# cfdeinza/reinforcement-learning-rendezvous

Hardware: AMD Instinct MI355X
Metric: env steps/sec (higher is better)
Workload: dtype f64

## Files before the change

### reinforcement_learning_rendezvous_amd/csrc/rdv_policy.h

```cpp
#pragma once

#include <hip/hip_runtime.h>
#include <stdint.h>

#include <cmath>
#include <cstring>
#include <vector>

#include "rdv_device.h"

namespace rdv {

constexpr int kPolIn = 17, kPolHid = 64, kPolOut = 6;
constexpr int kPolWaveEnvs = 32;
constexpr int kPolBlock = 512;
constexpr int kPolBlockEnvs = (kPolBlock / 64) * kPolWaveEnvs;

typedef float f32x16 __attribute__((ext_vector_type(16)));
typedef float pol_f4 __attribute__((ext_vector_type(4)));
typedef float pol_f2 __attribute__((ext_vector_type(2)));
typedef _Float16 f16x8 __attribute__((ext_vector_type(8)));

constexpr int kPolXShift = 10;
constexpr int kPolFragBytes = 64 * 16;
constexpr int kPolW1Frag = 0, kPolW2Frag = 8, kPolW3Frag = 24, kPolFrags = 32;
constexpr int kPolF32 = kPolFrags * kPolFragBytes / 4;
constexpr int kPolB1 = kPolF32, kPolB2 = kPolB1 + 64, kPolB3 = kPolB2 + 64, kPolStd = kPolB3 + 32, kPolLogStd = kPolStd + 8,
              kPolScale = kPolLogStd + 8, kPolFloats = kPolScale + 4;
static_assert(kPolFloats % 4 == 0, "the parameter block is copied as float4");
constexpr int kPolObsStage = kPolWaveEnvs * kPolIn, kPolActStage = kPolWaveEnvs * kPolOut;
constexpr int kPolLdsBytes = (kPolFloats + (kPolBlock / 64) * (kPolObsStage + kPolActStage)) * 4;

inline uint16_t pol_f16_rn(float x) {
  uint32_t u; std::memcpy(&u, &x, 4);
  const uint32_t sign = (u >> 16) & 0x8000u;
  const uint32_t a = u & 0x7fffffffu;
  if (a > 0x7f800000u) return (uint16_t)(sign | 0x7e00u);
  if (a >= 0x477ff000u) return (uint16_t)(sign | 0x7c00u);
  if (a < 0x33000001u) return (uint16_t)sign;
  int e = (int)(a >> 23) - 127;
  uint32_t m = (a & 0x7fffffu) | 0x800000u;
  int shift = e >= -14 ? 13 : 13 + (-14 - e);
  uint32_t q = m >> shift;
  const uint32_t rem = m & ((1u << shift) - 1u), half = 1u << (shift - 1);
  if (rem > half || (rem == half && (q & 1u))) ++q;
  uint32_t out = e >= -14 ? (uint32_t)((e + 15) << 10) + (q - 0x400u) : q;
  return (uint16_t)(sign | out);
}
inline float pol_f16_f(uint16_t hbits) {
  const uint32_t sign = (uint32_t)(hbits & 0x8000u) << 16, e = (hbits >> 10) & 0x1fu, m = hbits & 0x3ffu;
  float mag;
  if (e == 0) mag = std::ldexp((float)m, -24);
  else if (e == 31) mag = m ? NAN : INFINITY;
  else mag = std::ldexp((float)(m | 0x400u), (int)e - 25);
  return sign ? -mag : mag;
}
inline int pol_layer_shift(const float* wts, int count) {
  float mx = 0.0f;
  for (int i = 0; i < count; ++i) mx = std::fmax(mx, std::fabs(wts[i]));
  int sft = 10;
  while (sft > -20 && std::ldexp(mx, sft) >= 32768.0f) --sft;
  return sft;
}
inline void pol_put(uint16_t* frags, int frag0, int mt_count, int ks_count, int mt, int ks, int lane, int j, float wv, int sft) {
  const float ws = std::ldexp(wv, sft);
  const uint16_t hi = pol_f16_rn(ws);
  const uint16_t term[2] = {hi, pol_f16_rn(ws - pol_f16_f(hi))};
  for (int q = 0; q < 2; ++q) frags[((size_t)(frag0 + (q * mt_count + mt) * ks_count + ks) * 64 + (size_t)lane) * 8 + (size_t)j] = term[q];
}

inline void pack_policy_weights(const float* w1, const float* b1, const float* w2, const float* b2, const float* w3, const float* b3,
                                const float* log_std, int out_dim, std::vector<float>& packed) {
  packed.assign((size_t)kPolFloats, 0.0f);
  uint16_t* frags = reinterpret_cast<uint16_t*>(packed.data());
  const int sh1 = pol_layer_shift(w1, kPolHid * kPolIn), sh2 = pol_layer_shift(w2, kPolHid * kPolHid), sh3 = pol_layer_shift(w3, out_dim * kPolHid);
  auto put = [&](int frag0, int mt_count, int ks_count, int mt, int ks, int lane, int j, float wv, int sft) {
    pol_put(frags, frag0, mt_count, ks_count, mt, ks, lane, j, wv, sft);
  };
  for (int lane = 0; lane < 64; ++lane) {
    const int r = lane & 31, h = lane >> 5;
    for (int j = 0; j < 8; ++j) {
      for (int mt = 0; mt < 2; ++mt) {
        for (int s = 0; s < 2; ++s) {
          const int k = 16 * s + 8 * h + j;
          put(kPolW1Frag, 2, 2, mt, s, lane, j, k < kPolIn ? w1[(32 * mt + r) * kPolIn + k] : 0.0f, sh1);
        }
        for (int ks = 0; ks < 4; ++ks) {
          const int k = 32 * (ks >> 1) + 16 * (ks & 1) + 8 * (j >> 2) + 4 * h + (j & 3);
          put(kPolW2Frag, 2, 4, mt, ks, lane, j, w2[(32 * mt + r) * kPolHid + k], sh2);
        }
      }
      for (int ks = 0; ks < 4; ++ks) {
        const int k = 32 * (ks >> 1) + 16 * (ks & 1) + 8 * (j >> 2) + 4 * h + (j & 3);
        put(kPolW3Frag, 1, 4, 0, ks, lane, j, r < out_dim ? w3[r * kPolHid + k] : 0.0f, sh3);
      }
    }
  }
  const float acc1 = std::ldexp(1.0f, kPolXShift + sh1), acc2 = std::ldexp(1.0f, kPolXShift + sh2), acc3 = std::ldexp(1.0f, kPolXShift + sh3);
  for (int mt = 0; mt < 2; ++mt)
    for (int h = 0; h < 2; ++h)
      for (int e = 0; e < 16; ++e) {
        const int row = (e & 3) + 8 * (e >> 2) + 4 * h;
        packed[kPolB1 + (mt * 2 + h) * 16 + e] = b1[32 * mt + row] * acc1;
        packed[kPolB2 + (mt * 2 + h) * 16 + e] = b2[32 * mt + row] * acc2;
        if (mt == 0) packed[kPolB3 + h * 16 + e] = row < out_dim ? b3[row] * acc3 : 0.0f;
      }
  packed[kPolScale + 0] = 1.0f / acc1; packed[kPolScale + 1] = 1.0f / acc2; packed[kPolScale + 2] = 1.0f / acc3;
  if (log_std) for (int j = 0; j < out_dim; ++j) { packed[kPolStd + j] = std::exp(log_std[j]); packed[kPolLogStd + j] = log_std[j]; }
}

__device__ __forceinline__ void tanh2_f32(float x0, float x1, float kexp, float& t0, float& t1) {
  const pol_f2 x = {x0, x1};
  const pol_f2 y = x * kexp;
  const pol_f2 e = {__builtin_amdgcn_exp2f(y.x), __builtin_amdgcn_exp2f(y.y)};
  const pol_f2 s1 = e + 1.0f;
  const pol_f2 r = {__builtin_amdgcn_rcpf(s1.x), __builtin_amdgcn_rcpf(s1.y)};
  constexpr float one = (float)(1 << kPolXShift);
  const pol_f2 t = __builtin_elementwise_fma(pol_f2{-2.0f * one, -2.0f * one}, r, pol_f2{one, one});
  t0 = t.x; t1 = t.y;
}

__device__ __forceinline__ void box_muller(uint32_t a, uint32_t b, float& n0, float& n1) {
  const float u1 = ((float)(a >> 8) + 0.5f) * (1.0f / 16777216.0f);
  const float u2 = ((float)(b >> 8) + 0.5f) * (1.0f / 16777216.0f);
  const float r = sqrtf(-2.0f * __logf(u1));
  float s, c;
  __sincosf(6.28318530717958647692f * u2, &s, &c);
  n0 = r * c; n1 = r * s;
}

__device__ __forceinline__ void wave_fence() {
  __builtin_amdgcn_fence(__ATOMIC_ACQ_REL, "wavefront");
  __builtin_amdgcn_wave_barrier();
}

typedef _Float16 pol_h2 __attribute__((ext_vector_type(2)));
__device__ __forceinline__ void split2(const float (&x)[8], f16x8 (&t)[2]) {
  uint32_t hi[4], lo[4];
#pragma unroll
  for (int p = 0; p < 4; ++p) {
    const pol_f2 v = {x[2 * p], x[2 * p + 1]};
    const pol_h2 h = __builtin_convertvector(v, pol_h2);
    __builtin_memcpy(&hi[p], &h, 4);
  }
  asm("v_fma_mixlo_f16 %0, %4, 1.0, -%12 op_sel_hi:[0,0,1]\n\t"
      "v_fma_mixlo_f16 %1, %6, 1.0, -%13 op_sel_hi:[0,0,1]\n\t"
      "v_fma_mixlo_f16 %2, %8, 1.0, -%14 op_sel_hi:[0,0,1]\n\t"
      "v_fma_mixlo_f16 %3, %10, 1.0, -%15 op_sel_hi:[0,0,1]\n\t"
      "v_fma_mixhi_f16 %0, %5, 1.0, -%12 op_sel:[0,0,1] op_sel_hi:[0,0,1]\n\t"
      "v_fma_mixhi_f16 %1, %7, 1.0, -%13 op_sel:[0,0,1] op_sel_hi:[0,0,1]\n\t"
      "v_fma_mixhi_f16 %2, %9, 1.0, -%14 op_sel:[0,0,1] op_sel_hi:[0,0,1]\n\t"
      "v_fma_mixhi_f16 %3, %11, 1.0, -%15 op_sel:[0,0,1] op_sel_hi:[0,0,1]\n\t"
      "s_nop 0"
      : "=&v"(lo[0]), "=&v"(lo[1]), "=&v"(lo[2]), "=&v"(lo[3])
      : "v"(x[0]), "v"(x[1]), "v"(x[2]), "v"(x[3]), "v"(x[4]), "v"(x[5]), "v"(x[6]), "v"(x[7]), "v"(hi[0]), "v"(hi[1]), "v"(hi[2]), "v"(hi[3]));
#pragma unroll
  for (int p = 0; p < 4; ++p) {
    pol_h2 h, l;
    __builtin_memcpy(&h, &hi[p], 4);
    __builtin_memcpy(&l, &lo[p], 4);
    t[0][2 * p] = h.x; t[0][2 * p + 1] = h.y; t[1][2 * p] = l.x; t[1][2 * p + 1] = l.y;
  }
}

__device__ __forceinline__ f32x16 mfma3(const f16x8 (&a)[2], const f16x8 (&b)[2], f32x16 d) {
  d = __builtin_amdgcn_mfma_f32_32x32x16_f16(a[1], b[0], d, 0, 0, 0);
  d = __builtin_amdgcn_mfma_f32_32x32x16_f16(a[0], b[1], d, 0, 0, 0);
  d = __builtin_amdgcn_mfma_f32_32x32x16_f16(a[0], b[0], d, 0, 0, 0);
  return d;
}

template <int MT, int KS>
__device__ __forceinline__ void layer(const float* w, int frag0, const float* biasp, const f16x8 (&xb)[KS][2], int lane, f32x16 (&d)[MT]) {
  const f16x8* wf = reinterpret_cast<const f16x8*>(w) + lane;
  const int h = lane >> 5;
#pragma unroll
  for (int mt = 0; mt < MT; ++mt)
#pragma unroll
    for (int e4 = 0; e4 < 4; ++e4) {
      const float4 b = *reinterpret_cast<const float4*>(biasp + (mt * 2 + h) * 16 + 4 * e4);
      d[mt][4 * e4 + 0] = b.x; d[mt][4 * e4 + 1] = b.y; d[mt][4 * e4 + 2] = b.z; d[mt][4 * e4 + 3] = b.w;
    }
#pragma unroll
  for (int mt = 0; mt < MT; ++mt)
#pragma unroll
    for (int ks = 0; ks < KS; ++ks) {
      f16x8 a[2];
#pragma unroll
      for (int q = 0; q < 2; ++q) a[q] = wf[(frag0 + (q * MT + mt) * KS + ks) * 64];
      d[mt] = mfma3(a, xb[ks], d[mt]);
    }
}

__device__ __forceinline__ void activate(const f32x16& d, float kexp, f16x8 (&lo_step)[2], f16x8 (&hi_step)[2]) {
  float x[8];
#pragma unroll
  for (int j = 0; j < 8; j += 2) tanh2_f32(d[j], d[j + 1], kexp, x[j], x[j + 1]);
  split2(x, lo_step);
#pragma unroll
  for (int j = 0; j < 8; j += 2) tanh2_f32(d[8 + j], d[9 + j], kexp, x[j], x[j + 1]);
  split2(x, hi_step);
}

__device__ __forceinline__ void actor_inputs(const float* rows, int lane, f16x8 (&x0)[2][2]) {
  const int r = lane & 31, h = lane >> 5;
  const float* row = rows + r * kPolIn;
  constexpr float xs = (float)(1 << kPolXShift), xmax = 63.0f * xs;
  auto in = [&](float v) { const float c = __builtin_amdgcn_fmed3f(v * xs, -xmax, xmax); return v != v ? v : c; };
  {
    float x[8];
#pragma unroll
    for (int j = 0; j < 8; ++j) x[j] = in(row[8 * h + j]);
    split2(x, x0[0]);
    const float last = in(row[16]);
#pragma unroll
    for (int j = 0; j < 8; ++j) x[j] = 0.0f;
    x[0] = h == 0 ? last : 0.0f;
    split2(x, x0[1]);
  }
}

__device__ __forceinline__ void actor_means(const float* w, const float* rows, int lane, float (&mean)[4]) {
  f16x8 x0[2][2];
  actor_inputs(rows, lane, x0);
  constexpr float two_log2e = 2.8853900817779268f;
  f32x16 d1[2];
  layer<2, 2>(w, kPolW1Frag, w + kPolB1, x0, lane, d1);
  f16x8 x1[4][2];
  const float k1 = two_log2e * w[kPolScale + 0];
  activate(d1[0], k1, x1[0], x1[1]);
  activate(d1[1], k1, x1[2], x1[3]);
  f32x16 d2[2];
  layer<2, 4>(w, kPolW2Frag, w + kPolB2, x1, lane, d2);
  f16x8 x2[4][2];
  const float k2 = two_log2e * w[kPolScale + 1];
  activate(d2[0], k2, x2[0], x2[1]);
  activate(d2[1], k2, x2[2], x2[3]);
  f32x16 d3[1];
  layer<1, 4>(w, kPolW3Frag, w + kPolB3, x2, lane, d3);
  const float s3 = w[kPolScale + 2];
  mean[0] = d3[0][0] * s3; mean[1] = d3[0][1] * s3; mean[2] = d3[0][2] * s3; mean[3] = d3[0][3] * s3;
}

__device__ __forceinline__ void actor_noise(int lane, uint64_t seed, uint64_t id, uint64_t counter, float (&z)[4]) {
  const int h = lane >> 5;
  uint32_t c0 = (uint32_t)id, c1 = (uint32_t)(id >> 32), c2 = (uint32_t)counter, c3 = (uint32_t)(counter >> 32) * 2u + (uint32_t)h;
  philox4x32_10(c0, c1, c2, c3, (uint32_t)seed, (uint32_t)(seed >> 32) ^ 0x504F4C49u);
  box_muller(c0, c1, z[0], z[1]);
  box_muller(c2, c3, z[2], z[3]);
}

__device__ __forceinline__ float actor_apply_at(const float* sd, int lane, const float (&z)[4], float (&a)[4]) {
  const int h = lane >> 5;
  float lp = 0.0f;
#pragma unroll
  for (int c = 0; c < 4; ++c) {
    const bool valid = h == 0 || c < 2;
    a[c] = fmaf(sd[4 * h + c], z[c], a[c]);
    lp += valid ? fmaf(-0.5f * z[c], z[c], -sd[kPolLogStd - kPolStd + 4 * h + c]) : 0.0f;
  }
  return (lp + __shfl_xor(lp, 32)) - 5.5136312f;
}
__device__ __forceinline__ float actor_apply(const float* w, int lane, const float (&z)[4], float (&a)[4]) {
  return actor_apply_at(w + kPolStd, lane, z, a);
}
__device__ __forceinline__ float actor_sample_at(const float* sd, int lane, int deterministic, uint64_t seed, uint64_t id, uint64_t counter,
                                                 float (&a)[4]) {
  float z[4] = {0.0f, 0.0f, 0.0f, 0.0f};
  if (!deterministic) actor_noise(lane, seed, id, counter, z);
  return actor_apply_at(sd, lane, z, a);
}

__device__ __forceinline__ float clip_action(float v) { return (v != v) ? v : fminf(fmaxf(v, -1.0f), 1.0f); }

__device__ __forceinline__ void stage_obs_rows(const float* __restrict__ obs, int64_t wave_base, int64_t nrows, float* rows, int lane) {
  if (nrows > 0) {
    const float* src = obs + wave_base * kPolIn;
    if (nrows == kPolWaveEnvs) {
#pragma unroll
      for (int k = 0; k < 3; ++k) {
        const int q = k * 64 + lane;
        if (q < kPolObsStage / 4)
          *reinterpret_cast<pol_f4*>(rows + 4 * q) = __builtin_nontemporal_load(reinterpret_cast<const pol_f4*>(src + 4 * q));
      }
    } else {
      const int64_t valid = nrows * kPolIn;
      for (int j = 0; j < 9; ++j) {
        const int idx = j * 64 + lane;
        if (idx < kPolObsStage) rows[idx] = idx < valid ? src[idx] : 0.0f;
      }
    }
  }
}

__device__ __forceinline__ void actor_outputs(const float* sd, int lane, int64_t wave_base, int64_t nrows, int deterministic, uint64_t seed,
                                              uint64_t counter, uint64_t env_id_offset, float (&a)[4], float* arows, float* __restrict__ actions,
                                              float* __restrict__ raw_actions, float* __restrict__ log_prob) {
  const int r = lane & 31, h = lane >> 5;
  const float logp = actor_sample_at(sd, lane, deterministic, seed, env_id_offset + (uint64_t)(wave_base + r), counter, a);
  if (log_prob && h == 0 && r < nrows) log_prob[wave_base + r] = logp;
  if (raw_actions && r < nrows) {
    float* dst = raw_actions + (wave_base + r) * kPolOut + 4 * h;
    dst[0] = a[0]; dst[1] = a[1];
    if (h == 0) { dst[2] = a[2]; dst[3] = a[3]; }
  }

  if (h == 0) {
#pragma unroll
    for (int c = 0; c < 4; ++c) arows[r * kPolOut + c] = clip_action(a[c]);
  } else {
    arows[r * kPolOut + 4] = clip_action(a[0]);
    arows[r * kPolOut + 5] = clip_action(a[1]);
  }
  wave_fence();
  {
    float* dst = actions + wave_base * kPolOut;
    const int64_t valid = nrows * kPolOut;
#pragma unroll
    for (int k = 0; k < 2; ++k) {
      const int idx = k * 128 + lane * 2;
      if (idx + 1 < valid) {
        *reinterpret_cast<float2*>(dst + idx) = *reinterpret_cast<const float2*>(arows + idx);
      } else if (idx < valid) {
        dst[idx] = arows[idx];
      }
    }
  }
}

#ifndef RDV_POLICY_FUNCTIONS_ONLY
__global__ __launch_bounds__(kPolBlock) void policy_act_kernel(const float* __restrict__ W, const float* __restrict__ obs,
                                                               float* __restrict__ actions, int64_t n, int deterministic,
                                                               uint64_t seed, uint64_t counter, uint64_t env_id_offset,
                                                               float* __restrict__ raw_actions, float* __restrict__ log_prob) {
  extern __shared__ __attribute__((aligned(16))) float lds[];
  float* w = lds;
  const int lane = threadIdx.x & 63;
  const int wv = threadIdx.x >> 6;
  float* rows = lds + kPolFloats + wv * kPolObsStage;
  float* arows = lds + kPolFloats + (kPolBlock / 64) * kPolObsStage + wv * kPolActStage;
  const int64_t wave_base = ((int64_t)blockIdx.x * (kPolBlock / 64) + wv) * kPolWaveEnvs;
  const int64_t nrows = (n - wave_base) < kPolWaveEnvs ? (n - wave_base) : kPolWaveEnvs;

#ifndef RDV_POL_NOSTAGE
  for (int q = threadIdx.x; q < kPolFloats / 4; q += kPolBlock)
    *reinterpret_cast<float4*>(w + 4 * q) = *reinterpret_cast<const float4*>(W + 4 * q);
#endif

  stage_obs_rows(obs, wave_base, nrows, rows, lane);
  __syncthreads();
  if (nrows <= 0) return;

  float a[4];
  if (wv < 4) __builtin_amdgcn_s_setprio(1);
  actor_means(w, rows, lane, a);
  if (wv < 4) __builtin_amdgcn_s_setprio(0);
  actor_outputs(w + kPolStd, lane, wave_base, nrows, deterministic, seed, counter, env_id_offset, a, arows, actions, raw_actions, log_prob);
}

__global__ __launch_bounds__(kPolBlock) void policy_value_kernel(const float* __restrict__ W, const float* __restrict__ obs,
                                                                 float* __restrict__ values, int64_t n) {
  extern __shared__ __attribute__((aligned(16))) float lds[];
  float* w = lds;
  const int lane = threadIdx.x & 63;
  const int wv = threadIdx.x >> 6;
  float* rows = lds + kPolFloats + wv * kPolObsStage;
  const int64_t wave_base = ((int64_t)blockIdx.x * (kPolBlock / 64) + wv) * kPolWaveEnvs;
  const int64_t nrows = (n - wave_base) < kPolWaveEnvs ? (n - wave_base) : kPolWaveEnvs;
  for (int q = threadIdx.x; q < kPolFloats / 4; q += kPolBlock)
    *reinterpret_cast<float4*>(w + 4 * q) = *reinterpret_cast<const float4*>(W + 4 * q);
  stage_obs_rows(obs, wave_base, nrows, rows, lane);
  __syncthreads();
  if (nrows <= 0) return;
  float v[4];
  actor_means(w, rows, lane, v);
  if (lane < nrows) values[wave_base + lane] = v[0];
}
#endif

}
```

### reinforcement_learning_rendezvous_amd/csrc/rdv_policy_mlp.h

```cpp
#pragma once

#include "rdv_policy.h"
#include "../../include/rdv.h"

namespace rdv {

constexpr float kMlpSigmoidAbsErr = 2.0e-7f;
constexpr int kMlpLayers = RDV_MLP_MAX_HIDDEN + 1;
constexpr int kMlpRec = 8, kMlpRecStride = 8, kMlpStd = 48, kMlpZero = 64, kMlpHdr = 128;
static_assert(kPolLogStd - kPolStd == 8, "actor_apply_at reads log_std 8 floats behind exp(log_std)");
constexpr int kMlpStageFloats = (kPolBlock / 64) * (kPolObsStage + kPolActStage);
constexpr int kMlpMaxFloats = kMlpHdr + (8 + 3 * 16 + 8) * (kPolFragBytes / 4) + (4 * 2 + 1) * 32;
constexpr int kMlpMaxLdsBytes = (kMlpMaxFloats + kMlpStageFloats) * 4;
static_assert(kMlpMaxLdsBytes <= 160 * 1024, "the largest network's workgroup must fit the CU's 160 KiB of LDS");
inline int mlp_lds_bytes(int block_floats) { return (block_floats + kMlpStageFloats) * 4; }

inline int mlp_tiles(int width) { return width == 64 ? 2 : 1; }
inline int mlp_ksteps(int width) { return width / 16; }

inline void pack_mlp_weights(const RdvMlpSpec& spec, int out_dim, const float* const* weights, const float* const* biases,
                             const float* log_std, std::vector<float>& packed) {
  const int L = spec.n_hidden;
  int frag0[kMlpLayers], mt_n[kMlpLayers], ks_n[kMlpLayers], in_w[kMlpLayers], out_w[kMlpLayers], frags_total = 0, tiles_total = 0;
  for (int l = 0; l <= L; ++l) {
    in_w[l] = l == 0 ? kPolIn : spec.hidden[l - 1];
    out_w[l] = l < L ? spec.hidden[l] : out_dim;
    mt_n[l] = l < L ? mlp_tiles(out_w[l]) : 1;
    ks_n[l] = l == 0 ? 2 : mlp_ksteps(in_w[l]);
    frag0[l] = frags_total;
    frags_total += 2 * mt_n[l] * ks_n[l];
    tiles_total += mt_n[l];
  }
  const int bias0 = kMlpHdr + frags_total * (kPolFragBytes / 4);
  const int total = bias0 + tiles_total * 32;
  packed.assign((size_t)total, 0.0f);
  int32_t* hdr = reinterpret_cast<int32_t*>(packed.data());
  hdr[0] = L; hdr[1] = spec.activation; hdr[2] = out_dim; hdr[3] = total;
  uint16_t* frags = reinterpret_cast<uint16_t*>(packed.data() + kMlpHdr);
  int bias_at = bias0;
  for (int l = 0; l <= L; ++l) {
    const float* wl = weights[l];
    const int sft = pol_layer_shift(wl, out_w[l] * in_w[l]);
    for (int lane = 0; lane < 64; ++lane) {
      const int r = lane & 31, h = lane >> 5;
      for (int j = 0; j < 8; ++j)
        for (int mt = 0; mt < mt_n[l]; ++mt)
          for (int ks = 0; ks < ks_n[l]; ++ks) {
            const int k = l == 0 ? 16 * ks + 8 * h + j : 32 * (ks >> 1) + 16 * (ks & 1) + 8 * (j >> 2) + 4 * h + (j & 3);
            const int row = 32 * mt + r;
            pol_put(frags, frag0[l], mt_n[l], ks_n[l], mt, ks, lane, j, (row < out_w[l] && k < in_w[l]) ? wl[row * in_w[l] + k] : 0.0f, sft);
          }
    }
    const float acc = std::ldexp(1.0f, kPolXShift + sft);
    for (int mt = 0; mt < mt_n[l]; ++mt)
      for (int h = 0; h < 2; ++h)
        for (int e = 0; e < 16; ++e) {
          const int row = 32 * mt + (e & 3) + 8 * (e >> 2) + 4 * h;
          packed[(size_t)(bias_at + (mt * 2 + h) * 16 + e)] = row < out_w[l] ? biases[l][row] * acc : 0.0f;
        }
    int32_t* rec = hdr + kMlpRec + kMlpRecStride * l;
    rec[0] = frag0[l]; rec[1] = bias_at; rec[2] = mt_n[l]; rec[3] = ks_n[l];
    packed[(size_t)(kMlpRec + kMlpRecStride * l + 4)] = 1.0f / acc;
    bias_at += mt_n[l] * 32;
  }
  if (log_std) for (int j = 0; j < out_dim; ++j) { packed[kMlpStd + j] = std::exp(log_std[j]); packed[kMlpStd + 8 + j] = log_std[j]; }
}

hipError_t mlp_raise_lds_limit();
void mlp_launch_act(int activation, const float* W, int block_floats, const float* obs, float* actions, int64_t n, int deterministic,
                    uint64_t seed, uint64_t counter, uint64_t env_id_offset, float* raw_actions, float* log_prob, hipStream_t s);
void mlp_launch_value(int activation, const float* W, int block_floats, const float* obs, float* values, int64_t n, hipStream_t s);

template <int ACT>
__device__ __forceinline__ float mlp_act_const(float inv) {
  if (ACT == RDV_ACT_TANH) return 2.8853900817779268f * inv;
  if (ACT == RDV_ACT_SIGMOID) return -1.4426950408889634f * inv;
  return inv * (float)(1 << kPolXShift);
}

template <int ACT>
__device__ __forceinline__ void mlp_act2(float x0, float x1, float k, float& t0, float& t1) {
  constexpr float one = (float)(1 << kPolXShift);
  if (ACT == RDV_ACT_TANH) {
    tanh2_f32(x0, x1, k, t0, t1);
  } else if (ACT == RDV_ACT_SIGMOID) {
    const pol_f2 y = pol_f2{x0, x1} * k;
    const pol_f2 e = {__builtin_amdgcn_exp2f(y.x), __builtin_amdgcn_exp2f(y.y)};
    const pol_f2 s1 = e + 1.0f;
    const pol_f2 r = {__builtin_amdgcn_rcpf(s1.x), __builtin_amdgcn_rcpf(s1.y)};
    const pol_f2 t = r * one;
    t0 = t.x; t1 = t.y;
  } else {
    const pol_f2 v = pol_f2{x0, x1} * k;
    const float c0 = __builtin_amdgcn_fmed3f(v.x, 0.0f, 63.0f * one), c1 = __builtin_amdgcn_fmed3f(v.y, 0.0f, 63.0f * one);
    t0 = v.x != v.x ? v.x : c0; t1 = v.y != v.y ? v.y : c1;
  }
}

template <int ACT>
__device__ __forceinline__ void mlp_activate(const f32x16& d, float k, f16x8 (&lo_step)[2], f16x8 (&hi_step)[2]) {
  float x[8];
#pragma unroll
  for (int j = 0; j < 8; j += 2) mlp_act2<ACT>(d[j], d[j + 1], k, x[j], x[j + 1]);
  split2(x, lo_step);
#pragma unroll
  for (int j = 0; j < 8; j += 2) mlp_act2<ACT>(d[8 + j], d[9 + j], k, x[j], x[j + 1]);
  split2(x, hi_step);
}

__device__ __forceinline__ void mlp_add_bias(f32x16& d, const float* b16) {
#pragma unroll
  for (int e4 = 0; e4 < 4; ++e4) {
    const float4 b = *reinterpret_cast<const float4*>(b16 + 4 * e4);
    d[4 * e4 + 0] += b.x; d[4 * e4 + 1] += b.y; d[4 * e4 + 2] += b.z; d[4 * e4 + 3] += b.w;
  }
}

template <int ACT, int MT, int KS>
__device__ __forceinline__ void mlp_hidden(const float* wf, const float* zerop, int frag0, const float* biasp, float k, int lane, f16x8 (&x)[4][2]) {
  f16x8 xin[KS][2];
#pragma unroll
  for (int ks = 0; ks < KS; ++ks) { xin[ks][0] = x[ks][0]; xin[ks][1] = x[ks][1]; }
  f32x16 d[MT];
  layer<MT, KS>(wf, frag0, zerop, xin, lane, d);
#pragma unroll
  for (int mt = 0; mt < MT; ++mt) {
    mlp_add_bias(d[mt], biasp + (mt * 2 + (lane >> 5)) * 16);
    mlp_activate<ACT>(d[mt], k, x[2 * mt], x[2 * mt + 1]);
  }
}

template <int KS>
__device__ __forceinline__ void mlp_head(const float* wf, const float* zerop, int frag0, const float* biasp, float inv, int lane, const f16x8 (&x)[4][2], float (&mean)[4]) {
  f16x8 xin[KS][2];
#pragma unroll
  for (int ks = 0; ks < KS; ++ks) { xin[ks][0] = x[ks][0]; xin[ks][1] = x[ks][1]; }
  f32x16 d[1];
  layer<1, KS>(wf, frag0, zerop, xin, lane, d);
  const float4 b = *reinterpret_cast<const float4*>(biasp + (lane >> 5) * 16);
  d[0][0] += b.x; d[0][1] += b.y; d[0][2] += b.z; d[0][3] += b.w;
  mean[0] = d[0][0] * inv; mean[1] = d[0][1] * inv; mean[2] = d[0][2] * inv; mean[3] = d[0][3] * inv;
}

template <int ACT>
__device__ __forceinline__ void mlp_means(const float* w, const int32_t* __restrict__ H, const float* rows, int lane, float (&mean)[4]) {
  const float* wf = w + kMlpHdr;
  const float* zerop = w + kMlpZero;
  const int L = H[0];
  f16x8 x[4][2];
  {
    f16x8 x0[2][2];
    actor_inputs(rows, lane, x0);
#pragma unroll
    for (int q = 0; q < 2; ++q) { x[0][q] = x0[0][q]; x[1][q] = x0[1][q]; x[2][q] = (f16x8)(0); x[3][q] = (f16x8)(0); }
  }
#pragma nounroll
  for (int l = 0; l < L; ++l) {
    const int32_t* rec = H + kMlpRec + kMlpRecStride * l;
    const int frag0 = rec[0];
    const float* biasp = w + rec[1];
    const float k = mlp_act_const<ACT>(__int_as_float(rec[4]));
    switch (rec[2] * 8 + rec[3]) {
      case 8 + 1: mlp_hidden<ACT, 1, 1>(wf, zerop, frag0, biasp, k, lane, x); break;
      case 8 + 2: mlp_hidden<ACT, 1, 2>(wf, zerop, frag0, biasp, k, lane, x); break;
      case 8 + 4: mlp_hidden<ACT, 1, 4>(wf, zerop, frag0, biasp, k, lane, x); break;
      case 16 + 1: mlp_hidden<ACT, 2, 1>(wf, zerop, frag0, biasp, k, lane, x); break;
      case 16 + 2: mlp_hidden<ACT, 2, 2>(wf, zerop, frag0, biasp, k, lane, x); break;
      default: mlp_hidden<ACT, 2, 4>(wf, zerop, frag0, biasp, k, lane, x); break;
    }
  }
  const int32_t* rec = H + kMlpRec + kMlpRecStride * L;
  const int frag0 = rec[0];
  const float* biasp = w + rec[1];
  const float inv = __int_as_float(rec[4]);
  switch (rec[3]) {
    case 1: mlp_head<1>(wf, zerop, frag0, biasp, inv, lane, x, mean); break;
    case 2: mlp_head<2>(wf, zerop, frag0, biasp, inv, lane, x, mean); break;
    default: mlp_head<4>(wf, zerop, frag0, biasp, inv, lane, x, mean); break;
  }
}

template <int ACT, bool CRITIC>
__global__ __launch_bounds__(kPolBlock) __attribute__((amdgpu_waves_per_eu(4))) void mlp_kernel(const float* __restrict__ W, const float* __restrict__ obs, float* __restrict__ out,
                                                        int64_t n, int deterministic, uint64_t seed, uint64_t counter, uint64_t env_id_offset,
                                                        float* __restrict__ raw_actions, float* __restrict__ log_prob) {
  extern __shared__ __attribute__((aligned(16))) float lds[];
  const int32_t* H = reinterpret_cast<const int32_t*>(W);
  const int total = H[3];
  float* w = lds;
  const int lane = threadIdx.x & 63;
  const int wv = threadIdx.x >> 6;
  float* rows = lds + total + wv * kPolObsStage;
  float* arows = lds + total + (kPolBlock / 64) * kPolObsStage + wv * kPolActStage;
  const int64_t wave_base = ((int64_t)blockIdx.x * (kPolBlock / 64) + wv) * kPolWaveEnvs;
  const int64_t nrows = (n - wave_base) < kPolWaveEnvs ? (n - wave_base) : kPolWaveEnvs;
  for (int q = threadIdx.x; q < total / 4; q += kPolBlock)
    *reinterpret_cast<float4*>(w + 4 * q) = *reinterpret_cast<const float4*>(W + 4 * q);
  stage_obs_rows(obs, wave_base, nrows, rows, lane);
  __syncthreads();
  if (nrows <= 0) return;
  float a[4];
  mlp_means<ACT>(w, H, rows, lane, a);
  if (CRITIC) {
    if (lane < nrows) out[wave_base + lane] = a[0];
  } else {
    actor_outputs(w + kMlpStd, lane, wave_base, nrows, deterministic, seed, counter, env_id_offset, a, arows, out, raw_actions, log_prob);
  }
}

}
```

Before: 10.35 billion.

## Split weight staging so layer-2/3 fragments load while layer 1 computes

Splits the LDS weight staging of the policy kernels into an early part (layer-1 fragments, f32 params, observations) and a late part (layer-2/3 fragments). All global loads are issued up front into registers. Only the early part is stored before the first barrier, and the late fragments are written to LDS after layer 1 runs, behind a second barrier. Full observation tiles are now loaded with nontemporal vector loads. The aim is to hide global-load latency behind layer-1 MFMA work, at the cost of more live registers and an extra block barrier.

```diff
diff --git a/reinforcement_learning_rendezvous_amd/csrc/rdv_policy.h b/reinforcement_learning_rendezvous_amd/csrc/rdv_policy.h
--- a/reinforcement_learning_rendezvous_amd/csrc/rdv_policy.h
+++ b/reinforcement_learning_rendezvous_amd/csrc/rdv_policy.h
@@ -220,10 +220,34 @@
   }
 }
 
+constexpr float kPolTwoLog2e = 2.8853900817779268f;
+__device__ __forceinline__ void actor_layer1(const float* w, const float* rows, int lane, f32x16 (&d1)[2]) {
+  f16x8 x0[2][2];
+  actor_inputs(rows, lane, x0);
+  layer<2, 2>(w, kPolW1Frag, w + kPolB1, x0, lane, d1);
+}
+__device__ __forceinline__ void actor_activate1(const float* w, const f32x16 (&d1)[2], f16x8 (&x1)[4][2]) {
+  const float k1 = kPolTwoLog2e * w[kPolScale + 0];
+  activate(d1[0], k1, x1[0], x1[1]);
+  activate(d1[1], k1, x1[2], x1[3]);
+}
+__device__ __forceinline__ void actor_rest(const float* w, const f16x8 (&x1)[4][2], int lane, float (&mean)[4]) {
+  constexpr float two_log2e = kPolTwoLog2e;
+  f32x16 d2[2];
+  layer<2, 4>(w, kPolW2Frag, w + kPolB2, x1, lane, d2);
+  f16x8 x2[4][2];
+  const float k2 = two_log2e * w[kPolScale + 1];
+  activate(d2[0], k2, x2[0], x2[1]);
+  activate(d2[1], k2, x2[2], x2[3]);
+  f32x16 d3[1];
+  layer<1, 4>(w, kPolW3Frag, w + kPolB3, x2, lane, d3);
+  const float s3 = w[kPolScale + 2];
+  mean[0] = d3[0][0] * s3; mean[1] = d3[0][1] * s3; mean[2] = d3[0][2] * s3; mean[3] = d3[0][3] * s3;
+}
 __device__ __forceinline__ void actor_means(const float* w, const float* rows, int lane, float (&mean)[4]) {
   f16x8 x0[2][2];
   actor_inputs(rows, lane, x0);
-  constexpr float two_log2e = 2.8853900817779268f;
+  constexpr float two_log2e = kPolTwoLog2e;
   f32x16 d1[2];
   layer<2, 2>(w, kPolW1Frag, w + kPolB1, x0, lane, d1);
   f16x8 x1[4][2];
@@ -328,6 +352,64 @@
   }
 }
 
+constexpr int kPolEarly4 = kPolW2Frag * kPolFragBytes / 16;
+constexpr int kPolLatePerThread = (kPolFrags - kPolW2Frag) * kPolFragBytes / 16 / kPolBlock;
+constexpr int kPolF32Quads = (kPolFloats - kPolF32) / 4;
+static_assert(kPolEarly4 == kPolBlock && kPolLatePerThread * kPolBlock * 4 == kPolF32 - kPolEarly4 * 4 && kPolF32Quads <= kPolBlock,
+              "one early and kPolLatePerThread late float4 of fragments per thread");
+struct PolStaged {
+  float4 frag1, f32s;
+  pol_f4 obs[3];
+  float4 late[kPolLatePerThread];
+};
+__device__ __forceinline__ void stage_issue(const float* __restrict__ W, const float* __restrict__ obs, int64_t wave_base, int64_t nrows,
+                                            int lane, PolStaged& st) {
+  const float4* W4 = reinterpret_cast<const float4*>(W);
+  const int t = threadIdx.x;
+#ifndef RDV_POL_NOSTAGE
+  st.frag1 = W4[t];
+  st.f32s = W4[kPolF32 / 4 + (t < kPolF32Quads ? t : kPolF32Quads - 1)];
+#endif
+  if (nrows == kPolWaveEnvs) {
+    const pol_f4* src = reinterpret_cast<const pol_f4*>(obs + wave_base * kPolIn);
+#pragma unroll
+    for (int k = 0; k < 3; ++k) {
+      const int q = k * 64 + lane;
+      st.obs[k] = __builtin_nontemporal_load(src + (q < kPolObsStage / 4 ? q : kPolObsStage / 4 - 1));
+    }
+  }
+#ifndef RDV_POL_NOSTAGE
+  __builtin_amdgcn_sched_barrier(0);
+#pragma unroll
+  for (int k = 0; k < kPolLatePerThread; ++k) st.late[k] = W4[kPolEarly4 + k * kPolBlock + t];
+#endif
+}
+__device__ __forceinline__ void stage_early_store(float* w, const float* __restrict__ obs, int64_t wave_base, int64_t nrows, float* rows,
+                                                  int lane, const PolStaged& st) {
+  const int t = threadIdx.x;
+#ifndef RDV_POL_NOSTAGE
+  reinterpret_cast<float4*>(w)[t] = st.frag1;
+  const bool own = t < kPolF32Quads;
+  const float4 second = {own ? st.f32s.x : st.frag1.x, own ? st.f32s.y : st.frag1.y, own ? st.f32s.z : st.frag1.z, own ? st.f32s.w : st.frag1.w};
+  reinterpret_cast<float4*>(w)[own ? kPolF32 / 4 + t : t] = second;
+#endif
+  if (nrows == kPolWaveEnvs) {
+#pragma unroll
+    for (int k = 0; k < 3; ++k) {
+      const int q = k * 64 + lane;
+      if (q < kPolObsStage / 4) *reinterpret_cast<pol_f4*>(rows + 4 * q) = st.obs[k];
+    }
+  } else {
+    stage_obs_rows(obs, wave_base, nrows, rows, lane);
+  }
+}
+__device__ __forceinline__ void stage_late_store(float* w, const PolStaged& st) {
+#ifndef RDV_POL_NOSTAGE
+#pragma unroll
+  for (int k = 0; k < kPolLatePerThread; ++k) reinterpret_cast<float4*>(w)[kPolEarly4 + k * kPolBlock + threadIdx.x] = st.late[k];
+#endif
+}
+
 #ifndef RDV_POLICY_FUNCTIONS_ONLY
 __global__ __launch_bounds__(kPolBlock) void policy_act_kernel(const float* __restrict__ W, const float* __restrict__ obs,
                                                                float* __restrict__ actions, int64_t n, int deterministic,
@@ -342,18 +424,24 @@
   const int64_t wave_base = ((int64_t)blockIdx.x * (kPolBlock / 64) + wv) * kPolWaveEnvs;
   const int64_t nrows = (n - wave_base) < kPolWaveEnvs ? (n - wave_base) : kPolWaveEnvs;
 
-#ifndef RDV_POL_NOSTAGE
-  for (int q = threadIdx.x; q < kPolFloats / 4; q += kPolBlock)
-    *reinterpret_cast<float4*>(w + 4 * q) = *reinterpret_cast<const float4*>(W + 4 * q);
-#endif
-
-  stage_obs_rows(obs, wave_base, nrows, rows, lane);
+  PolStaged st;
+  stage_issue(W, obs, wave_base, nrows, lane, st);
+  stage_early_store(w, obs, wave_base, nrows, rows, lane, st);
   __syncthreads();
-  if (nrows <= 0) return;
+  const bool live = nrows > 0;
+  f32x16 d1[2];
+  if (live) {
+    if (wv < 4) __builtin_amdgcn_s_setprio(1);
+    actor_layer1(w, rows, lane, d1);
+  }
+  stage_late_store(w, st);
+  f16x8 x1[4][2];
+  if (live) actor_activate1(w, d1, x1);
+  __syncthreads();
+  if (!live) return;
 
   float a[4];
-  if (wv < 4) __builtin_amdgcn_s_setprio(1);
-  actor_means(w, rows, lane, a);
+  actor_rest(w, x1, lane, a);
   if (wv < 4) __builtin_amdgcn_s_setprio(0);
   actor_outputs(w + kPolStd, lane, wave_base, nrows, deterministic, seed, counter, env_id_offset, a, arows, actions, raw_actions, log_prob);
 }
@@ -367,13 +455,20 @@
   float* rows = lds + kPolFloats + wv * kPolObsStage;
   const int64_t wave_base = ((int64_t)blockIdx.x * (kPolBlock / 64) + wv) * kPolWaveEnvs;
   const int64_t nrows = (n - wave_base) < kPolWaveEnvs ? (n - wave_base) : kPolWaveEnvs;
-  for (int q = threadIdx.x; q < kPolFloats / 4; q += kPolBlock)
-    *reinterpret_cast<float4*>(w + 4 * q) = *reinterpret_cast<const float4*>(W + 4 * q);
-  stage_obs_rows(obs, wave_base, nrows, rows, lane);
+  PolStaged st;
+  stage_issue(W, obs, wave_base, nrows, lane, st);
+  stage_early_store(w, obs, wave_base, nrows, rows, lane, st);
   __syncthreads();
-  if (nrows <= 0) return;
+  const bool live = nrows > 0;
+  f32x16 d1[2];
+  if (live) actor_layer1(w, rows, lane, d1);
+  stage_late_store(w, st);
+  f16x8 x1[4][2];
+  if (live) actor_activate1(w, d1, x1);
+  __syncthreads();
+  if (!live) return;
   float v[4];
-  actor_means(w, rows, lane, v);
+  actor_rest(w, x1, lane, v);
   if (lane < nrows) values[wave_base + lane] = v[0];
 }
 #endif
diff --git a/reinforcement_learning_rendezvous_amd/csrc/rdv_policy_mlp.h b/reinforcement_learning_rendezvous_amd/csrc/rdv_policy_mlp.h
--- a/reinforcement_learning_rendezvous_amd/csrc/rdv_policy_mlp.h
+++ b/reinforcement_learning_rendezvous_amd/csrc/rdv_policy_mlp.h
@@ -194,8 +194,10 @@
   float* arows = lds + total + (kPolBlock / 64) * kPolObsStage + wv * kPolActStage;
   const int64_t wave_base = ((int64_t)blockIdx.x * (kPolBlock / 64) + wv) * kPolWaveEnvs;
   const int64_t nrows = (n - wave_base) < kPolWaveEnvs ? (n - wave_base) : kPolWaveEnvs;
+#ifndef RDV_POL_NOSTAGE
   for (int q = threadIdx.x; q < total / 4; q += kPolBlock)
     *reinterpret_cast<float4*>(w + 4 * q) = *reinterpret_cast<const float4*>(W + 4 * q);
+#endif
   stage_obs_rows(obs, wave_base, nrows, rows, lane);
   __syncthreads();
   if (nrows <= 0) return;
```

Result: no change. 10.32 billion (-0.4%).
